# catniplab/vjf

Measured on AMD Instinct MI355X. Metric: trial-timesteps/sec, higher is better.
Workload: dtype f32

## Files before the change

include/vjf_hip.h:

```cpp
#ifndef VJF_HIP_H
#define VJF_HIP_H

#include <stdint.h>

#ifdef __cplusplus
extern "C" {
#endif

#define VJF_ABI_VERSION 1
#define VJF_MAX_HIDDEN 8

#define VJF_LIK_GAUSSIAN 0
#define VJF_LIK_POISSON 1

#define VJF_FLAG_SGD 1u
#define VJF_FLAG_UPDATE 2u
#define VJF_FLAG_WARM_UP 4u
#define VJF_FLAG_EXACT_NONFINITE 8u

#define VJF_STATUS_NONFINITE_RECON 1u
#define VJF_STATUS_NONFINITE_DYN 2u
#define VJF_STATUS_NONFINITE_ENT 4u
#define VJF_STATUS_RLS_FAILED 8u
#define VJF_STATUS_WAIT_RESIDENT 0x100u
// ... 137 lines not shown
int vjf_smooth_sample(const float* mu, const float* logvar, const float* u, const float* centroid, const float* logwidth,
                      const float* w_mean, const float* noise, const float* after, float* x,
                      int32_t T, int32_t S, int32_t B, int32_t n, int32_t d, int32_t dout, float state_var, void* stream);
int vjf_kstep_score_scratch_size(int32_t T, int32_t B, int32_t K, int32_t dout, int32_t dy, int64_t* bytes);
int vjf_kstep_score_plan(int32_t T, int32_t B, int32_t K, int32_t n, int32_t d, int32_t dout, int32_t dy, int64_t* lds_bytes,
                         int64_t* tiles, int64_t* tiles_per_chunk, int32_t* forms);
int vjf_kstep_score(const float* mu, const float* y, const float* u, const float* centroid, const float* logwidth,
                    const float* w_mean, const float* dec_W, const float* dec_b, double* sse_x, double* base_x, double* sse_y,
                    double* base_y, float* pred, void* scratch, int32_t T, int32_t B, int32_t K, int32_t n, int32_t d, int32_t dout,
                    int32_t dy, int32_t poisson, void* stream);
int vjf_ekf_plan(int32_t n, int32_t d, int32_t dout, int32_t dy, int64_t* lds_bytes);
int vjf_ekf(const float* y, const float* u, const uint8_t* observed, const float* centroid, const float* logwidth,
            const float* w_mean, const float* dec_W, const float* dec_b, const float* prior_mean, const float* prior_logvar,
            const float* prior_cov, float* mean, float* var, float* cov, float* loglik, float* cov_last, int32_t T, int32_t B,
            int32_t n, int32_t d, int32_t dout, int32_t dy, float state_var, float obs_var, void* stream);
int vjf_rls_scratch_size(int32_t B, int32_t n, int32_t dout, int64_t* bytes);
int vjf_blr_rls(const float* x, const float* target, const float* v, float shrink, const float* centroid,
                const float* logwidth, float* w_mean, float* w_chol, float* w_precision, float* w_pchol,
                void* scratch, uint32_t* status, int32_t B, int32_t n, int32_t d, int32_t dout, void* stream);

int vjf_kalman_scratch_size(int32_t B, int32_t n, int32_t dout, int64_t* bytes);
int vjf_blr_kalman(const float* x, const float* target, const float* v, float diffusion, const float* centroid,
                   const float* logwidth, float* w_mean, float* w_chol, void* scratch, uint32_t* status, int32_t B,
                   int32_t n, int32_t d, int32_t dout, void* stream);
int vjf_recognition_forward(const float* y, const float* u, const float* mu_s, const float* lv_s,
                            const float* const* rec_W, const float* const* rec_b, const float* mean_W,
                            const float* lv_W, const float* lv_b, float* mu_t, float* lv_t, int32_t B,
                            int32_t ydim, int32_t udim, int32_t xdim, int32_t n_hidden,
                            const int32_t* hidden, void* stream);
int vjf_recognition_forward_act(const float* y, const float* u, const float* mu_s, const float* lv_s,
// ... 16 lines not shown
```

vjf_amd/_native.py:

```python
import ctypes as C
import os

HERE = os.path.dirname(os.path.abspath(__file__))
_variant = os.environ.get("VJF_LIB", "")
LIB_PATH = os.path.join(HERE, f"libvjf_hip_{_variant}.so" if _variant.isalnum() else "libvjf_hip.so")

ABI_VERSION = 1
MAX_HIDDEN = 8
LIK_GAUSSIAN, LIK_POISSON = 0, 1
FLAG_SGD, FLAG_UPDATE, FLAG_WARM_UP, FLAG_EXACT_NONFINITE = 1, 2, 4, 8
STATUS_NONFINITE_RECON, STATUS_NONFINITE_DYN, STATUS_NONFINITE_ENT, STATUS_RLS_FAILED = 1, 2, 4, 8
STATUS_NOT_RESIDENT, STATUS_WAIT_MASK = 0x20000, 0x3ff00

SLOT_PRIOR_MEAN, SLOT_PRIOR_LOGVAR, SLOT_LIK_LOGVAR, SLOT_TR_LOGVAR, SLOT_CENTROID, SLOT_LOGWIDTH = range(6)
SLOT_REC_W0, SLOT_REC_B0 = 6, 7
SLOT_MEAN_W, SLOT_LV_W, SLOT_LV_B, SLOT_DEC_W, SLOT_DEC_B = 22, 23, 24, 25, 26
SLOT_W_MEAN, SLOT_W_CHOL, SLOT_W_PREC, SLOT_W_PCHOL, SLOT_SCALARS = 27, 28, 29, 30, 31
N_SLOTS = 32
SC_N_LIK, SC_N_TR, SC_LR_LIK, SC_LR_DEC, SC_LR_TR, SC_LR_REC, SC_FREEZE_DEC, SC_STATUS, SC_TRI_CLEAN, SC_SHRINK = range(10)
N_SCALARS = 16


ACT_TANH, ACT_RELU, ACT_LEAKY_RELU, ACT_ELU, ACT_SOFTPLUS, ACT_SIGMOID, ACT_HARDTANH = range(7)

# ... 48 lines not shown
    "vjf_forecast_ens_chunks": [_I, _I, _I, _I, _I, C.POINTER(_I), C.POINTER(_I)],
    "vjf_forecast_ens": [_P, C.c_int64] + [_P] * 16 + [_I] * 7 + [_P],
    "vjf_tangent_plan": [_I, _I, _I, _I, C.POINTER(_I), C.POINTER(C.c_int64)],
    "vjf_tangent_rollout": [_P] * 10 + [_I] * 8 + [_P],
    "vjf_fixed_points_plan": [_I, _I, _I, C.POINTER(C.c_int64)],
    "vjf_fixed_points": [_P] * 10 + [_I] * 5 + [_F, _F, _P],
    "vjf_smooth_plan": [_I, _I, _I, C.POINTER(C.c_int64)],
    "vjf_smooth": [_P] * 12 + [_I] * 5 + [_F, _P],
    "vjf_smooth_sample_plan": [_I, _I, _I, _I, C.POINTER(_I), C.POINTER(C.c_int64)],
    "vjf_smooth_sample": [_P] * 9 + [_I] * 6 + [_F, _P],
    "vjf_kstep_score_scratch_size": [_I, _I, _I, _I, _I, C.POINTER(C.c_int64)],
    "vjf_kstep_score_plan": [_I] * 7 + [C.POINTER(C.c_int64)] * 3 + [C.POINTER(_I)],
    "vjf_kstep_score": [_P] * 14 + [_I] * 8 + [_P],
    "vjf_ekf_plan": [_I, _I, _I, _I, C.POINTER(C.c_int64)],
    "vjf_ekf": [_P] * 16 + [_I] * 6 + [_F, _F, _P],
    "vjf_rls_scratch_size": [_I, _I, _I, C.POINTER(C.c_int64)],
    "vjf_blr_rls": [_P, _P, _P, _F, _P, _P, _P, _P, _P, _P, _P, _P, _I, _I, _I, _I, _P],
    "vjf_kalman_scratch_size": [_I, _I, _I, C.POINTER(C.c_int64)],
    "vjf_blr_kalman": [_P, _P, _P, _F, _P, _P, _P, _P, _P, _P, _I, _I, _I, _I, _P],
    "vjf_recognition_forward": [_P, _P, _P, _P, C.POINTER(_P), C.POINTER(_P), _P, _P, _P, _P, _P, _I, _I, _I, _I, _I,
                                C.POINTER(_I), _P],
    "vjf_recognition_forward_act": [_P, _P, _P, _P, C.POINTER(_P), C.POINTER(_P), _P, _P, _P, _P, _P, _I, _I, _I, _I, _I,
                                    C.POINTER(_I), C.POINTER(VjfActivation), _P],
    "vjf_gaussian_loss": [_P, _P, _P, _P, _P, _P, _I, _I, _P],
    "vjf_gaussian_entropy": [_P, _P, _I, _I, _P],
    "vjf_poisson_loss": [_P, _P, _P, _I, _I, _P],
    "vjf_linear_forward": [_P, _P, _P, _P, _I, _I, _I, _P],
}

_lib = None
# ... 64 lines not shown
```

vjf_amd/csrc/vjf_abi.hip:

```cpp
#include <hip/hip_runtime.h>
#include <hip/hip_ext.h>

#include <dlfcn.h>

#include <cstdarg>
#include <cstdio>
#include <cstdlib>
#include <cstring>
#include <ctime>
#include <atomic>
#include <mutex>
#include <new>
#include <string>
#include <type_traits>
#include <vector>

#include "../../include/vjf_hip.h"
#include "vjf_chol_blocks.h"
#include "vjf_chol_kernel.h"
#include "vjf_gram_kernel.h"
#include "vjf_handoff.h"
#include "vjf_mega_kernel.h"
#include "vjf_ops_kernels.h"
#include "vjf_plan.h"
// ... 634 lines not shown
        return fail(-20, "vjf_ekf: bad shape (T=%d B=%d n=%d d=%d dout=%d dy=%d state_var=%g obs_var=%g%s)", T, B, n, d, dout, dy,
                    (double)state_var, (double)obs_var, !prior_logvar == !prior_cov ? ", exactly one of prior_logvar / prior_cov is needed" : "");
    if (d > dout && !u) return fail(-21, "vjf_ekf: u is required when d > dout");
    const EkfPlan p = ekf_plan(n, d, dout, dy, fc_env_on("VJF_FC_CENTROID_LDS"), fc_env_on("VJF_EKF_DECODER_LDS"));
    if (!p.fits)
        return fail(-11, "vjf_ekf: n=%d, d=%d, dout=%d beyond %s", n, d, dout,
                    dout > VJF_EKF_MAXDOUT ? "dout <= 32 (VJF_EKF_MAXDOUT)" : "one workgroup's LDS");
    VjfEkfArgs a{};
    a.y = y; a.u = d > dout ? u : nullptr; a.obs = observed; a.c = centroid; a.logw = logwidth; a.w = w_mean; a.dec_W = dec_W;
    a.dec_b = dec_b; a.prior_mean = prior_mean; a.prior_lv = prior_logvar; a.prior_cov = prior_cov; a.mean = mean; a.var = var;
    a.cov = cov; a.ll = loglik; a.cov_last = cov_last; a.T = T; a.B = B; a.n = n; a.d = d; a.dout = dout; a.dy = dy; a.q = state_var;
    a.r = obs_var;
    return ekf_run(a, p, (hipStream_t)stream);
}

int vjf_rls_scratch_size(int32_t B, int32_t n, int32_t dout, int64_t* bytes) {
    if (!bytes || B < 1 || n < 1 || dout < 1) return fail(-20, "vjf_rls_scratch_size: bad argument");
    *bytes = (int64_t)rls_carve(B, n, dout, nullptr).total;
    return 0;
}

int vjf_blr_rls(const float* x, const float* target, const float* v, float shrink, const float* centroid, const float* logwidth,
                float* w_mean, float* w_chol, float* w_precision, float* w_pchol, void* scratch, uint32_t* status, int32_t B,
                int32_t n, int32_t d, int32_t dout, void* stream) {
    if (!x || !target || !v || !centroid || !logwidth || !w_mean || !w_chol || !w_precision || !w_pchol || !scratch)
        return fail(-1, "vjf_blr_rls: null tensor");
    if (B < 1 || n < 1 || d < 1 || dout < 1) return fail(-20, "vjf_blr_rls: bad shape");
    return rls_update("vjf_blr_rls", "RLS kernel", vjf_rls_kernel, scratch, x, target, centroid, logwidth, B, n, d, dout, stream, [&](VjfRlsArgs& a, const RlsStats& st) {
        a.Pm = w_precision; a.Wm = w_mean; a.Wc = w_chol; a.Lm = w_pchol;
        a.G = st.red + st.P.red_G; a.FDX = st.red + st.P.red_FDX; a.v = v; a.work = (float*)(st.ws + st.c.work); a.status = status;
// ... 74 lines not shown
```

vjf_amd/csrc/vjf_mega_trial.h:

```cpp
#pragma once
#include "vjf_mega_common.h"

template <bool RLS, bool ACT = false>
__device__ __forceinline__ void vjf_mega_trial(const VjfPlan& P, const VjfMegaArgs& A, float* smem, const int wg, const VjfAct act = VjfAct{}) {
    constexpr int LD = VJF_MG_LD, NW = VJF_MG_WAVES, NT = VJF_MG_THREADS, TR = VJF_MG_TR;
    constexpr bool VSPLIT = RLS && !ACT;
    const int tid0 = threadIdx.x;
    const int dz = P.dz, dy = P.dy, du = P.du, n = P.n, din = P.din, dxu = P.dxu;
    const float* S = A.state;
    float* SCW = A.state + P.off[VJF_SLOT_SCALARS];
    const bool do_sgd = RLS || (A.flags & VJF_FLAG_SGD) != 0u, do_upd = RLS || (A.flags & VJF_FLAG_UPDATE) != 0u;
    const bool warm = !RLS && (A.flags & VJF_FLAG_WARM_UP) != 0u;
    constexpr bool mode_rls = RLS;
    const bool gated = RLS || do_sgd || do_upd;
    const bool want_resid = !RLS && do_upd && warm;
    const bool use_mom = !RLS && A.n_mom > 0;
    const unsigned m_dy = mg_magic(dy), m_dz = mg_magic(dz), m_du = mg_magic(du > 0 ? du : 1);
    const VjfMegaTrialLds Lo = vjf_mega_trial_lds<false>(P, A.lds_floats);
    const bool tl = Lo.theta != 0;
    float* s_cen = smem + Lo.cen; float* s_iw = smem + Lo.iw;
    float* s_in = smem + Lo.in; float* s_xu = smem + Lo.xu; float* s_phi = smem + Lo.phi; float* s_act = smem + Lo.act;
    float* s_dd = smem + Lo.dd;
    float* s_mu = smem + Lo.mu; float* s_lv = smem + Lo.lv; float* s_xt = smem + Lo.xt; float* s_e2 = smem + Lo.e2; float* s_pm = smem + Lo.pm;
    float* s_dmu = smem + Lo.dmu; float* s_dlv = smem + Lo.dlv; float* s_dx = smem + Lo.dx;
// ... 457 lines not shown
                else if (tid < ly + le) tp = en + min((tid - ly) * 32, nbn * dz - 1);
                else if (tid < ly + 2 * le) tp = en + sz + min((tid - ly - le) * 32, nbn * dz - 1);
                if (tp) touch = *tp;
            }
            if (tid == 0 && !replay && mode_rls) {
                float v = 0.f;
                for (int bb = 0; bb < TR; ++bb) v += s_sc[bb * RS_N + RS_SDX2];
                s_wg[RS_SDX2] += v;
                if (last) vjf_st_wt(early + (size_t)16 * ldn + RS_SDX2, s_wg[RS_SDX2]);
            }
            if (first) VJF_MG_STAMP(26);
            const bool fuse_fwd = first && last && !replay && !rls_in && s_wg[15] != 0.f;
            if (last && !replay && !fuse_fwd && mode_rls) vjf_wg_signal_wt(cnt + MG_C_FWD, tid);
            if (first) VJF_MG_STAMP(4);
            if (last) { VJF_MG_STAMPX(28, -1); VJF_MG_STAMPW(1); }
            float4 wv_late[2];
            bool warm_late = false;
            if (first && !rls_in) {
                if (!vjf_wg_wait_sc1<RLS ? VJF_POLL_SLEEP : VJF_POLL_SLEEP_LITE>(cnt + MG_C_PDONE, (unsigned)t * npost, tid, SCW + VJF_SC_STATUS, (A.flags & VJF_FLAG_HANDOFF_ACQUIRE) != 0u))
                    vjf_status_or(SCW + VJF_SC_STATUS, VJF_STATUS_RLS_FAILED | VJF_STATUS_WAIT_K1);
                if (vjf_abort_wg()) return;
                sig = vjf_ld_sc1(S + P.off[VJF_SLOT_TR_LOGVAR]);
                tri = vjf_ld_sc1(SCW + VJF_SC_TRI_CLEAN) != 0.f;
                if (fuse_fwd) {
                    vjf_chaos(tid, cnt + MG_C_FWD, 2);
                    asm volatile("s_waitcnt vmcnt(0)" ::: "memory");
                    __syncthreads();
                    if (tid == 0) __hip_atomic_fetch_add(cnt + MG_C_FWD, 1u, __ATOMIC_RELAXED, __HIP_MEMORY_SCOPE_AGENT);
                }
                mg_warm_issue(A.xt, P.n * P.n, wg, tid, wv_late);
// ... 20 lines not shown
            if (last && tid == 0 && !replay && mode_rls) __hip_atomic_fetch_add(cnt + MG_C_K1, 1u, __ATOMIC_RELAXED, __HIP_MEMORY_SCOPE_AGENT);
            if (RLS) moments_b();
            if (do_sgd)
            for (int e = tid; e < TR * (dz + 1); e += NT) {
                const int j = e >> 5, b = e & 31;
                if (b < nb) {
                    float* sv = A.pmsave + (size_t)(b0 + b) * (dz + 1) + j;
                    if (!replay) *sv = j < dz ? s_pm[j * LD + b] : s_plv[b];
                    else if (j < dz) s_pm[j * LD + b] = *sv;
                    else s_plv[b] = *sv;
                }
            }
            if (replay) { __syncthreads(); MG_PHASE(); }
            if (first) VJF_MG_STAMP(10);
            if (first) { VJF_MG_STAMP(6); VJF_MG_STAMPW(3); }
            {
                constexpr int LPT = NT / TR;
                const int b = tid / LPT, s = tid % LPT;
                const bool ok = b < nb;
                float lrec = 0.f, ssey = 0.f;
                if (P.lik == VJF_LIK_GAUSSIAN) {
                    const float p = expf(-0.5f * rho), e = expf(-rho);
                    for (int i = s; i < dy; i += LPT) {
                        const float seed = vjf_gauss_recon(s_in[i * LD + b], s_py[i * LD + b], rho, p, e, lrec, ssey);
                        s_dpy[i * LD + b] = (ok && m_r) ? seed : 0.f;
                    }
                } else {
                    for (int i = s; i < dy; i += LPT) {
                        const float seed = vjf_poisson_recon(s_in[i * LD + b], s_py[i * LD + b], lrec, ssey);
                        s_dpy[i * LD + b] = (ok && m_r) ? seed : 0.f;
                    }
                }
                lrec = group_sum<LPT>(lrec);
                ssey = group_sum<LPT>(ssey);
                float ldyn = 0.f, ent = 0.f, rsd = 0.f;
                {
                    const float p = expf(-0.5f * sig), e = expf(-sig), plv = s_plv[b];
                    for (int j = s; j < dz; j += LPT) {
                        if (want_resid) { const float r = s_dx[j * LD + b] - s_dmu[j * LD + b]; rsd = fmaf(r, r, rsd); }
                        const VjfDynSeed sd = vjf_dyn_term(s_pm[j * LD + b], s_mu[j * LD + b], s_lv[j * LD + b], plv, sig, p, e, !warm && m_d, m_h, ldyn, ent);
                        s_dmu[j * LD + b] = ok ? sd.dmu : 0.f;
                        s_dlv[j * LD + b] = ok ? sd.dlv : 0.f;
                    }
                }
                ldyn = group_sum<LPT>(ldyn);
                ent = group_sum<LPT>(ent);
                if (want_resid) rsd = group_sum<LPT>(rsd);
                if (s == 0) {
                    s_sc[b * RS_N + RS_RESID] = ok ? rsd : 0.f;
                    s_sc[b * RS_N + RS_LRECON] = ok ? lrec : 0.f;
                    s_sc[b * RS_N + RS_LDYN] = ok ? ldyn : 0.f;
                    s_sc[b * RS_N + RS_ENT] = ok ? ent : 0.f;
                    s_sc[b * RS_N + RS_SSEY] = ok ? ssey : 0.f;
                }
            }
            __syncthreads(); MG_PHASE();
            if (first) VJF_MG_STAMP(31);
#ifdef VJF_EXPERIMENT_SLOW_TRIAL
            { const unsigned long long t0_ = wall_clock64(); while (wall_clock64() - t0_ < VJF_EXPERIMENT_SLOW_TRIAL) __builtin_amdgcn_s_sleep(1); }
#endif
            if ((tid < RS_SDX2 || (tid == RS_RESID && want_resid)) && !replay) {
                float v = 0.f;
                for (int bb = 0; bb < TR; ++bb) v += s_sc[bb * RS_N + tid];
                s_wg[tid] += v;
            }
            if (do_sgd) {
            int gbase = 0;
            auto grad_tensor = [&](const float* D, int M, const float* Bact, int Kin, int blkid) {
                int b_off, b_ldm, b_rows;
                mg_slab_block(P, blkid, b_off, b_ldm, b_rows);
                const int ntm = (M + 15) >> 4, ntj = (Kin + 1 + 15) >> 4;
                const unsigned mj = mg_magic(ntj);
                for (int q = (wave - gbase) & (NW - 1); q < ntm * ntj; q += NW) {
                    const int tm = mg_div(q, mj), tj = q - tm * ntj;
                    mg_grad_tile(D, M, tm * 16, Bact, Kin, tj * 16, s_one, s_zero, late + b_off, b_ldm, b_rows, first, lane);
                }
                gbase += ntm * ntj;
            };
            {
                const float* C = S + P.off[VJF_SLOT_DEC_W];
                const int mt = (dz + 15) >> 4;
                float* s_kp = compact ? s_py : s_dd;
                const int rows_av = compact ? dy : Lo.nd * P.hmax;
                const int nslb = min(NW / mt, rows_av / (16 * mt));
                if (nslb >= 2) {
                    if (wave < mt * nslb) {
                        const int tt = wave / nslb, sl = wave - tt * nslb;
                        const int per = (((dy + 3) >> 2) + nslb - 1) / nslb * 4;
                        vjf_f32x4 acc0 = {0.f, 0.f, 0.f, 0.f}, acc1 = {0.f, 0.f, 0.f, 0.f};
                        if (tl) mg_mma2_lds<true>(acc0, acc1, smem + Lo.th_dec, Lo.th_ldd, dz, tt * 16, s_dpy, sl * per, min(dy, (sl + 1) * per), lane);
                        else mg_mma2(acc0, acc1, C, dz, dz, tt * 16, s_dpy, sl * per, min(dy, (sl + 1) * per), lane);
                        float* pr = s_kp + (size_t)((sl * mt + tt) * 16 + 4 * (lane >> 4)) * LD + (lane & 15);
#pragma unroll
                        for (int r = 0; r < 4; ++r) { pr[r * LD] = acc0[r]; pr[r * LD + 16] = acc1[r]; }
                    }
                    __syncthreads(); MG_PHASE();
                    for (int e = tid; e < TR * dz; e += NT) {
                        const int j = e >> 5, b = e & 31;
                        float a = 0.f;
                        for (int sl = 0; sl < nslb; ++sl) a += s_kp[(size_t)((sl * mt + (j >> 4)) * 16 + (j & 15)) * LD + b];
                        s_dmu[j * LD + b] += a;
                        s_dlv[j * LD + b] = fmaf(a * s_e2[j * LD + b], 0.5f * expf(0.5f * s_lv[j * LD + b]), s_dlv[j * LD + b]);
                    }
                } else
                for (int tt = wave; tt < mt; tt += NW) {
                    vjf_f32x4 acc0 = {0.f, 0.f, 0.f, 0.f}, acc1 = {0.f, 0.f, 0.f, 0.f};
                    if (tl) mg_mma2_lds<true>(acc0, acc1, smem + Lo.th_dec, Lo.th_ldd, dz, tt * 16, s_dpy, 0, dy, lane);
                    else mg_mma2(acc0, acc1, C, dz, dz, tt * 16, s_dpy, 0, dy, lane);
#pragma unroll
                    for (int r = 0; r < 4; ++r) {
                        const int j = tt * 16 + 4 * (lane >> 4) + r;
                        if (j < dz) {
#pragma unroll
                            for (int g = 0; g < 2; ++g) {
                                const int b = 16 * g + (lane & 15);
// ... 125 lines not shown
```

vjf_amd/csrc/vjf_post_kernel.h:

```cpp
#pragma once
#include <hip/hip_runtime.h>
#include "vjf_handoff.h"
#include "vjf_plan.h"
#include "vjf_chol_kernel.h"
#include "vjf_trial_mfma_kernel.h"

#define VJF_POST_THREADS 512
#define VJF_POST_KPAR 4
#define VJF_POST_LDB 33
#define VJF_POST_LDX 17
#define VJF_RESID_BLOCKS 64

struct VjfPostArgs {
    float* state;
    const float* dinv;
    const float* lscr;
    const float* gbuf;
    const unsigned* flags;
    unsigned epoch;
    float* status;
    const unsigned* k1_done;
    unsigned k1_target;
    unsigned* started;
    unsigned* done;
// ... 15 lines not shown
#define VJF_POST_STAMP(i)                                                                   \
    do {                                                                                    \
        if (A.stamps && solve && tid == 0) {                                                \
            unsigned long long t_;                                                          \
            asm volatile("s_memrealtime %0\n\ts_waitcnt lgkmcnt(0)" : "=s"(t_)::"memory");      \
            A.stamps[((it_epoch & 7u) << 5) * (A.nsteps > 0 ? 1 : 0) + (i)] = t_;              \
        }                                                                                   \
    } while (0)

static inline size_t vjf_post_inv_lds_bytes(const VjfPlan& P) {
    const int nbl = (P.n + 31) / 32;
    return ((size_t)nbl * 32 * VJF_POST_LDB + (size_t)nbl * 32 * VJF_POST_LDX + 32 * VJF_POST_LDX + 64 + 16 + 16) * 4;
}
static inline size_t vjf_post_lds_bytes(const VjfPlan& P) {
    const int nbl = (P.n + 31) / 32;
    return ((size_t)(nbl * (nbl - 1) / 2 + nbl) * 32 * VJF_POST_LDB + (size_t)nbl * 32 * VJF_POST_LDX + 32 * VJF_POST_LDX + 64 + 16 + 16) * 4;
}

template <class FA>
__device__ __forceinline__ void post_mma32(vjf_f32x4& acc, const float* Bs, int lane, FA fa) {
    const int i = lane & 15, kk = lane >> 4;
    float a[8], b[8];
#pragma unroll
    for (int s = 0; s < 8; ++s) { a[s] = fa(i, 4 * s + kk); b[s] = Bs[(4 * s + kk) * VJF_POST_LDX + i]; }
    __builtin_amdgcn_sched_barrier(0);
    vjf_f32x4 acc1 = {0.f, 0.f, 0.f, 0.f};
#pragma unroll
    for (int s = 0; s < 8; s += 2) {
        acc = __builtin_amdgcn_mfma_f32_16x16x4f32(a[s], b[s], acc, 0, 0, 0);
        acc1 = __builtin_amdgcn_mfma_f32_16x16x4f32(a[s + 1], b[s + 1], acc1, 0, 0, 0);
    }
// ... 41 lines not shown

__device__ __forceinline__ void vjf_rls_post_body(const VjfPlan& P, const VjfPostArgs& A, float* lds, int* s_dead, const unsigned it_epoch,
                                                  const float* it_red, const unsigned it_k1_target, const unsigned it_prep_target,
                                                  const bool it_first, const int role, const int bix) {
    int tid = threadIdx.x;
    asm volatile("" : "+v"(tid));
    const int lane = tid & 63, wave = tid >> 6;
    const int n = P.n, dz = P.dz, nbl = (n + 31) / 32, ntri = nbl * (nbl + 1) / 2, nlow = ntri - nbl;
    const bool solve = role == 2 || bix == 2 * nbl;
    const bool col_only = role == 1;
    constexpr int LB = VJF_POST_LDB, LX = VJF_POST_LDX;
    float* s_L = lds;
    float* s_D = s_L + (size_t)(col_only ? nbl - 1 : nlow) * 32 * LB;
    float* s_x = s_D + (size_t)(col_only ? 1 : nbl) * 32 * LB;
    float* s_y = s_x + (size_t)nbl * 32 * LX;
    int* s_tab = reinterpret_cast<int*>(s_y + 32 * LX);
    int* s_ctl = s_tab + 64;
    auto leave = [&]() {
        vjf_chaos(tid, A.done, 2);
        asm volatile("s_waitcnt vmcnt(0)" ::: "memory");
        __syncthreads();
        if (A.stamps && !solve && tid == 0) {
            unsigned long long t_;
            asm volatile("s_memrealtime %0\n\ts_waitcnt lgkmcnt(0)" : "=s"(t_)::"memory");
            atomicMax(A.stamps + ((it_epoch & 7u) << 5) * (A.nsteps > 0 ? 1 : 0) + 22, t_);
        }
        if (tid == 0 && A.done) __hip_atomic_fetch_add(A.done, 1u, __ATOMIC_RELAXED, __HIP_MEMORY_SCOPE_AGENT);
    };
    const float* S = A.state;
    const __amdgpu_buffer_rsrc_t r_L = vjf_rsrc(A.lscr, (size_t)n * n), r_dinv = vjf_rsrc(A.dinv, (size_t)nbl * 1024);
    const int j0 = solve ? 0 : bix >> 1;
    const int c0 = solve ? 0 : 16 * (bix & 1);
    auto tri = [](int bi, int bj) { return bi * (bi - 1) / 2 + bj; };
    auto lblk = [&](int bi, int bj) { return s_L + (size_t)(col_only ? bi - bj - 1 : tri(bi, bj)) * 32 * LB; };
    auto dblk = [&](int k) { return s_D + (size_t)(col_only ? 0 : k) * 32 * LB; };

    if (tid == 0 && A.started && it_first) __hip_atomic_fetch_add(A.started, 1u, __ATOMIC_RELAXED, __HIP_MEMORY_SCOPE_AGENT);
    float pre_sdx2 = 0.f, pre_old = 0.f, pre_tot = 1.f;
    double pre_scale = 0.0;
    VJF_POST_STAMP(16);
    if (tid < ntri) {
        int bi = 0;
        while ((bi + 1) * (bi + 2) / 2 <= tid) ++bi;
        s_tab[32 + tid] = (bi << 8) | (tid - bi * (bi + 1) / 2);
    }
    if (!solve)
        for (int e = tid; e < nbl * 32 * 16; e += VJF_POST_THREADS) {
            const int r = e >> 4, c = e & 15;
            s_x[r * LX + c] = (r == j0 * 32 + c0 + c) ? 1.f : 0.f;
        }
    __syncthreads();

    float gpre[4][16], fpre[8];
    unsigned wbits[4];
    {
        const int c = lane & 31, h = lane >> 5;
#pragma unroll
        for (int q = 0; q < 4; ++q) {
            const int t = wave + 8 * q;
            unsigned wq = 0u;
            if (solve && t < ntri) {
                const int code = s_tab[32 + t], bi = code >> 8, bj = code & 255;
#pragma unroll
                for (int r = 0; r < 16; ++r) {
                    const int gi = bi * 32 + (r & 3) + 8 * (r >> 2) + 4 * h, gj = bj * 32 + c;
                    wq |= ((gi >= n || gj > gi) ? 0u : (gj == gi ? 1u : 2u)) << (2 * r);
                }
            }
            wbits[q] = wq;
        }
    }
    auto prefetch_G = [&]() {
        const float* G = it_red + P.red_G;
        const int c = lane & 31, h = lane >> 5;
#pragma unroll
        for (int q = 0; q < 4; ++q) {
            const int code = s_tab[32 + min(wave + 8 * q, ntri - 1)];
            const int bi = code >> 8, bj = code & 255;
#pragma unroll
            for (int r = 0; r < 16; ++r) {
                const int gi = min(bi * 32 + (r & 3) + 8 * (r >> 2) + 4 * h, n - 1), gj = min(bj * 32 + c, n - 1);
                gpre[q][r] = vjf_ld_sc1(G + (size_t)gi * n + gj);
            }
        }
    };
    auto prefetch_rest = [&]() {
        pre_sdx2 = vjf_ld_sc1(it_red + P.red_SC + RS_SDX2);
        const float sig = vjf_ld_sc1(S + P.off[VJF_SLOT_TR_LOGVAR]);
        const float Bf = (float)A.B_total;
        pre_old = vjf_running_old_share(sig, vjf_ld_sc1(S + P.off[VJF_SLOT_SCALARS] + VJF_SC_N_TR), VJF_TR_VAR_CAP, Bf, pre_tot);
        pre_scale = 1.0 / ((double)Bf * (double)P.dz);
        const float* FDX = it_red + P.red_FDX;
#pragma unroll
        for (int q = 0; q < 8; ++q) {
            const int e = tid + q * VJF_POST_THREADS, r = min(e >> 4, n - 1), cc = min(e & 15, dz - 1);
            fpre[q] = vjf_ld_sc1(FDX + r * dz + cc);
        }
    };
    auto prefetch_tail = [&]() { prefetch_G(); prefetch_rest(); };

    const int tile = wave & 1, grp = wave >> 1;
    const int xr = 4 * (lane >> 4), xc = lane & 15;
    int bad = 0;
    bool g_there = A.prep_count == nullptr;
    auto wait_g = [&]() {
        if (g_there) return;
        g_there = true;
        if (!vjf_wg_wait(A.prep_count, it_prep_target, tid, A.status)) { vjf_status_or(A.status, VJF_STATUS_RLS_FAILED | VJF_STATUS_WAIT_G); *s_dead = 1; }
    };
    auto stage_column = [&](int k) {
        const int nb = nbl - k;
        float4 v[4];
        const int r = (tid >> 3) & 31, c4 = (tid & 7) * 4, bh = tid >> 8;
#pragma unroll
// ... 126 lines not shown
                }
            }
            if (A.xt) {
                const int gc0 = j0 * 32 + c0;
                for (int e = tid; e < (n - first) * 4; e += VJF_POST_THREADS) {
                    const int i = first + (e >> 2), q = (e & 3) * 4;
                    if (gc0 + q < n) {
                        vjf_f32x4 o = {s_x[i * LX + q], s_x[i * LX + q + 1], s_x[i * LX + q + 2], s_x[i * LX + q + 3]};
                        vjf_st4_wt(A.xt + (size_t)i * n + gc0 + q, o);
                    }
                }
            }
            leave();
            return;
        }
        for (int k = nbl - 1; k >= 0; --k) {
            vjf_f32x4 w = {0.f, 0.f, 0.f, 0.f};
            if (wave < 2) {
                const float* Db = s_D + (size_t)k * 32 * LB;
                post_mma32(w, s_x + (size_t)k * 32 * LX, lane, [&](int i, int m) { return Db[m * LB + 16 * wave + i]; });
#pragma unroll
                for (int r = 0; r < 4; ++r) s_y[(16 * wave + xr + r) * LX + xc] = w[r];
            }
            __syncthreads();
            if (wave < 2) {
#pragma unroll
                for (int r = 0; r < 4; ++r) s_x[(k * 32 + 16 * wave + xr + r) * LX + xc] = w[r];
            }
            for (int i = k - 1 - grp; i >= 0; i -= VJF_POST_THREADS / 128) {
                const float* Lb = s_L + (size_t)tri(k, i) * 32 * LB;
                float* xt = s_x + ((size_t)i * 32 + 16 * tile + xr) * LX + xc;
                vjf_f32x4 acc;
#pragma unroll
                for (int r = 0; r < 4; ++r) acc[r] = xt[r * LX];
                post_mma32(acc, s_y, lane, [&](int ii, int m) { return -Lb[m * LB + 16 * tile + ii]; });
#pragma unroll
                for (int r = 0; r < 4; ++r) xt[r * LX] = acc[r];
            }
            __syncthreads();
        }
        VJF_POST_STAMP(19);
    }
    auto store_W = [&]() {
        float* Wm = A.state + P.off[VJF_SLOT_W_MEAN];
        for (int e = tid; e < n * 16; e += VJF_POST_THREADS) {
            const int r = e >> 4, c = e & 15;
            if (c < dz) __hip_atomic_store(Wm + r * dz + c, s_x[r * LX + c], __ATOMIC_RELAXED, __HIP_MEMORY_SCOPE_AGENT);
        }
    };
    if (!failed && !k1_late) store_W();
    if (!A.fold_sigma) { leave(); return; }
    {
// ... 3 lines not shown
            if (tid == 0) { __builtin_amdgcn_fence(__ATOMIC_ACQUIRE, "agent"); asm volatile("s_waitcnt vmcnt(0)" ::: "memory"); }
            __syncthreads();
            const float* Wold = A.state + P.off[VJF_SLOT_W_MEAN];
            for (int e = tid; e < nbl * 32 * 16; e += VJF_POST_THREADS) {
                const int r = e >> 4, c = e & 15;
                s_x[r * LX + c] = (r < n && c < dz) ? Wold[(size_t)r * dz + c] : 0.f;
            }
            prefetch_tail();
            if (A.undo_P) {
                float* Pm = A.state + P.off[VJF_SLOT_W_PREC];
                const float* G = it_red + P.red_G;
                const float inv_v = expf(-S[P.off[VJF_SLOT_TR_LOGVAR]]);
                const float lam = vjf_shrink_of(S[P.off[VJF_SLOT_SCALARS] + VJF_SC_SHRINK]);
                for (int e = tid; e < n * n; e += VJF_POST_THREADS) vjf_st_wt(Pm + e, __fdiv_rn(fmaf(-G[e], inv_v, Pm[e]), lam));
            }
        }
        __syncthreads();
        VJF_POST_STAMP(20);
#ifdef VJF_EXPERIMENT_SLOW_RLS
        { const unsigned long long t0_ = wall_clock64(); while (wall_clock64() - t0_ < VJF_EXPERIMENT_SLOW_RLS) __builtin_amdgcn_s_sleep(1); }
#endif
        double part = 0.0;
        const int c = lane & 31, h = lane >> 5;
#pragma unroll
        for (int q = 0; q < 4; ++q) {
            const int t = wave + 8 * q;
            if (t < ntri) {
                const int code = s_tab[32 + t], bi = code >> 8, bj = code & 255;
                vjf_f32x16 acc;
#pragma unroll
                for (int r = 0; r < 16; ++r) acc[r] = 0.f;
                float wa[8], wb[8];
#pragma unroll
                for (int k = 0; k < 8; ++k) {
                    wa[k] = s_x[(bi * 32 + c) * LX + 2 * k + h];
                    wb[k] = s_x[(bj * 32 + c) * LX + 2 * k + h];
                }
#pragma unroll
                for (int k = 0; k < 8; ++k)
                    if (2 * k < dz) acc = __builtin_amdgcn_mfma_f32_32x32x2f32(wa[k], wb[k], acc, 0, 0, 0);
                double tp = 0.0;
#pragma unroll
                for (int r = 0; r < 16; ++r) {
                    const float wgt = (float)((wbits[q] >> (2 * r)) & 3u);
                    tp += (double)((wgt * gpre[q][r]) * acc[r]);
                }
                part += tp;
            }
        }
#pragma unroll
        for (int q = 0; q < 8; ++q) {
            const int e = tid + q * VJF_POST_THREADS, r = e >> 4, cc = e & 15;
            if (r < n && cc < dz) part -= 2.0 * (double)s_x[r * LX + cc] * (double)fpre[q];
        }

#pragma unroll
        for (int o = 32; o > 0; o >>= 1) part += __shfl_xor(part, o, 64);
        if (lane == 0) s_p[wave] = part;
        __syncthreads();
        if (tid == 0) {
            double t = 0.0;
            for (int w = 0; w < VJF_POST_THREADS / 64; ++w) t += s_p[w];
            t += (double)pre_sdx2;
// ... 197 lines not shown
```

Baseline: 83.07 million.

## Overlap back-substitution with W·Wᵀ trace tiles and hoist recon seeding

Restructures the post kernel's block back-substitution. Two waves now run the critical diagonal chain: they compute the next y block early into a double buffer, and the other six waves perform the off-diagonal updates in parallel. The sigma-fold W·Wᵀ trace tiles are dealt statically to waves and computed as soon as their column block is final, with per-tile partials kept in LDS, instead of as a separate pass afterward. In the mega-trial kernel, recon seed computation and decoder-gradient partials are moved earlier so they run before the warm/rls section. The cost is extra LDS, more complex scheduling, and a new tile-deal ABI helper.

```diff
diff --git a/include/vjf_hip.h b/include/vjf_hip.h
--- a/include/vjf_hip.h
+++ b/include/vjf_hip.h
@@ -175,6 +175,7 @@
             const float* w_mean, const float* dec_W, const float* dec_b, const float* prior_mean, const float* prior_logvar,
             const float* prior_cov, float* mean, float* var, float* cov, float* loglik, float* cov_last, int32_t T, int32_t B,
             int32_t n, int32_t d, int32_t dout, int32_t dy, float state_var, float obs_var, void* stream);
+int vjf_post_tile_deal(int32_t nbl, int32_t* owner, int32_t* step, int32_t* slots);
 int vjf_rls_scratch_size(int32_t B, int32_t n, int32_t dout, int64_t* bytes);
 int vjf_blr_rls(const float* x, const float* target, const float* v, float shrink, const float* centroid,
                 const float* logwidth, float* w_mean, float* w_chol, float* w_precision, float* w_pchol,
diff --git a/vjf_amd/_native.py b/vjf_amd/_native.py
--- a/vjf_amd/_native.py
+++ b/vjf_amd/_native.py
@@ -86,6 +86,7 @@
     "vjf_kstep_score": [_P] * 14 + [_I] * 8 + [_P],
     "vjf_ekf_plan": [_I, _I, _I, _I, C.POINTER(C.c_int64)],
     "vjf_ekf": [_P] * 16 + [_I] * 6 + [_F, _F, _P],
+    "vjf_post_tile_deal": [_I, C.POINTER(_I), C.POINTER(_I), C.POINTER(_I)],
     "vjf_rls_scratch_size": [_I, _I, _I, C.POINTER(C.c_int64)],
     "vjf_blr_rls": [_P, _P, _P, _F, _P, _P, _P, _P, _P, _P, _P, _P, _I, _I, _I, _I, _P],
     "vjf_kalman_scratch_size": [_I, _I, _I, C.POINTER(C.c_int64)],
diff --git a/vjf_amd/csrc/vjf_abi.hip b/vjf_amd/csrc/vjf_abi.hip
--- a/vjf_amd/csrc/vjf_abi.hip
+++ b/vjf_amd/csrc/vjf_abi.hip
@@ -672,6 +672,22 @@
     return ekf_run(a, p, (hipStream_t)stream);
 }
 
+int vjf_post_tile_deal(int32_t nbl, int32_t* owner, int32_t* step, int32_t* slots) {
+    if (!owner || !step || !slots || nbl < 1 || nbl > VJF_POST_MAXBLK) return fail(-20, "vjf_post_tile_deal: bad argument");
+    for (int bi = 0; bi < nbl; ++bi)
+        for (int bj = 0; bj <= bi; ++bj) {
+            owner[bi * (bi + 1) / 2 + bj] = vjf_post_deal_owner(nbl, bi, bj);
+            step[bi * (bi + 1) / 2 + bj] = bj;
+        }
+    for (int w = 0; w < VJF_POST_WAVES; ++w) {
+        int code[VJF_POST_SLOTS];
+        const int cnt = vjf_post_deal_slots(nbl, w, code);
+        if (cnt > VJF_POST_SLOTS) return fail(-11, "vjf_post_tile_deal: wavefront %d has %d tiles at nbl=%d", w, cnt, nbl);
+        for (int q = 0; q < VJF_POST_SLOTS; ++q) slots[w * VJF_POST_SLOTS + q] = code[q];
+    }
+    return 0;
+}
+
 int vjf_rls_scratch_size(int32_t B, int32_t n, int32_t dout, int64_t* bytes) {
     if (!bytes || B < 1 || n < 1 || dout < 1) return fail(-20, "vjf_rls_scratch_size: bad argument");
     *bytes = (int64_t)rls_carve(B, n, dout, nullptr).total;
diff --git a/vjf_amd/csrc/vjf_mega_trial.h b/vjf_amd/csrc/vjf_mega_trial.h
--- a/vjf_amd/csrc/vjf_mega_trial.h
+++ b/vjf_amd/csrc/vjf_mega_trial.h
@@ -5,6 +5,7 @@
 __device__ __forceinline__ void vjf_mega_trial(const VjfPlan& P, const VjfMegaArgs& A, float* smem, const int wg, const VjfAct act = VjfAct{}) {
     constexpr int LD = VJF_MG_LD, NW = VJF_MG_WAVES, NT = VJF_MG_THREADS, TR = VJF_MG_TR;
     constexpr bool VSPLIT = RLS && !ACT;
+    constexpr bool PRE = RLS && !ACT;
     const int tid0 = threadIdx.x;
     const int dz = P.dz, dy = P.dy, du = P.du, n = P.n, din = P.din, dxu = P.dxu;
     const float* S = A.state;
@@ -495,6 +496,66 @@
             if (last && !replay && !fuse_fwd && mode_rls) vjf_wg_signal_wt(cnt + MG_C_FWD, tid);
             if (first) VJF_MG_STAMP(4);
             if (last) { VJF_MG_STAMPX(28, -1); VJF_MG_STAMPW(1); }
+            auto recon_seeds = [&]() {
+                constexpr int LPT = NT / TR;
+                const int b = tid / LPT, s = tid % LPT;
+                const bool ok = b < nb;
+                float lrec = 0.f, ssey = 0.f;
+                if (P.lik == VJF_LIK_GAUSSIAN) {
+                    const float p = expf(-0.5f * rho), e = expf(-rho);
+                    for (int i = s; i < dy; i += LPT) {
+                        const float seed = vjf_gauss_recon(s_in[i * LD + b], s_py[i * LD + b], rho, p, e, lrec, ssey);
+                        s_dpy[i * LD + b] = (ok && m_r) ? seed : 0.f;
+                    }
+                } else {
+                    for (int i = s; i < dy; i += LPT) {
+                        const float seed = vjf_poisson_recon(s_in[i * LD + b], s_py[i * LD + b], lrec, ssey);
+                        s_dpy[i * LD + b] = (ok && m_r) ? seed : 0.f;
+                    }
+                }
+                lrec = group_sum<LPT>(lrec);
+                ssey = group_sum<LPT>(ssey);
+                if (s == 0) {
+                    s_sc[b * RS_N + RS_LRECON] = ok ? lrec : 0.f;
+                    s_sc[b * RS_N + RS_SSEY] = ok ? ssey : 0.f;
+                }
+            };
+            const int kp_mt = (dz + 15) >> 4;
+            float* s_kp = compact ? s_py : s_dd;
+            const int nslb = min(NW / kp_mt, (compact ? dy : Lo.nd * P.hmax) / (16 * kp_mt));
+            auto dpyc_partials = [&]() {
+                if (wave < kp_mt * nslb) {
+                    const float* C = S + P.off[VJF_SLOT_DEC_W];
+                    const int tt = wave / nslb, sl = wave - tt * nslb;
+                    const int per = (((dy + 3) >> 2) + nslb - 1) / nslb * 4;
+                    vjf_f32x4 acc0 = {0.f, 0.f, 0.f, 0.f}, acc1 = {0.f, 0.f, 0.f, 0.f};
+                    if (tl) mg_mma2_lds<true>(acc0, acc1, smem + Lo.th_dec, Lo.th_ldd, dz, tt * 16, s_dpy, sl * per, min(dy, (sl + 1) * per), lane);
+                    else mg_mma2(acc0, acc1, C, dz, dz, tt * 16, s_dpy, sl * per, min(dy, (sl + 1) * per), lane);
+                    float* pr = s_kp + (size_t)((sl * kp_mt + tt) * 16 + 4 * (lane >> 4)) * LD + (lane & 15);
+#pragma unroll
+                    for (int r = 0; r < 4; ++r) { pr[r * LD] = acc0[r]; pr[r * LD + 16] = acc1[r]; }
+                }
+            };
+            auto dpyc_sum = [&](int j, int b) {
+                float a = 0.f;
+                for (int sl = 0; sl < nslb; ++sl) a += s_kp[(size_t)((sl * kp_mt + (j >> 4)) * 16 + (j & 15)) * LD + b];
+                return a;
+            };
+            const bool pre = PRE && tl && Lo.part != Lo.dpy;
+            const bool pre_kp = pre && do_sgd && nslb >= 2;
+            if (pre) {
+                recon_seeds();
+                if (pre_kp) {
+                    __syncthreads(); MG_PHASE();
+                    dpyc_partials();
+                    __syncthreads(); MG_PHASE();
+                    for (int e = tid; e < TR * dz; e += NT) {
+                        const int j = e >> 5, b = e & 31;
+                        s_dx[j * LD + b] = dpyc_sum(j, b);
+                    }
+                    if (s_kp == s_part && !(first && !rls_in)) { __syncthreads(); MG_PHASE(); }
+                }
+            }
             float4 wv_late[2];
             bool warm_late = false;
             if (first && !rls_in) {
@@ -545,25 +606,11 @@
             if (replay) { __syncthreads(); MG_PHASE(); }
             if (first) VJF_MG_STAMP(10);
             if (first) { VJF_MG_STAMP(6); VJF_MG_STAMPW(3); }
+            if (!pre) recon_seeds();
             {
                 constexpr int LPT = NT / TR;
                 const int b = tid / LPT, s = tid % LPT;
                 const bool ok = b < nb;
-                float lrec = 0.f, ssey = 0.f;
-                if (P.lik == VJF_LIK_GAUSSIAN) {
-                    const float p = expf(-0.5f * rho), e = expf(-rho);
-                    for (int i = s; i < dy; i += LPT) {
-                        const float seed = vjf_gauss_recon(s_in[i * LD + b], s_py[i * LD + b], rho, p, e, lrec, ssey);
-                        s_dpy[i * LD + b] = (ok && m_r) ? seed : 0.f;
-                    }
-                } else {
-                    for (int i = s; i < dy; i += LPT) {
-                        const float seed = vjf_poisson_recon(s_in[i * LD + b], s_py[i * LD + b], lrec, ssey);
-                        s_dpy[i * LD + b] = (ok && m_r) ? seed : 0.f;
-                    }
-                }
-                lrec = group_sum<LPT>(lrec);
-                ssey = group_sum<LPT>(ssey);
                 float ldyn = 0.f, ent = 0.f, rsd = 0.f;
                 {
                     const float p = expf(-0.5f * sig), e = expf(-sig), plv = s_plv[b];
@@ -579,10 +626,8 @@
                 if (want_resid) rsd = group_sum<LPT>(rsd);
                 if (s == 0) {
                     s_sc[b * RS_N + RS_RESID] = ok ? rsd : 0.f;
-                    s_sc[b * RS_N + RS_LRECON] = ok ? lrec : 0.f;
                     s_sc[b * RS_N + RS_LDYN] = ok ? ldyn : 0.f;
                     s_sc[b * RS_N + RS_ENT] = ok ? ent : 0.f;
-                    s_sc[b * RS_N + RS_SSEY] = ok ? ssey : 0.f;
                 }
             }
             __syncthreads(); MG_PHASE();
@@ -610,26 +655,12 @@
             };
             {
                 const float* C = S + P.off[VJF_SLOT_DEC_W];
-                const int mt = (dz + 15) >> 4;
-                float* s_kp = compact ? s_py : s_dd;
-                const int rows_av = compact ? dy : Lo.nd * P.hmax;
-                const int nslb = min(NW / mt, rows_av / (16 * mt));
+                const int mt = kp_mt;
                 if (nslb >= 2) {
-                    if (wave < mt * nslb) {
-                        const int tt = wave / nslb, sl = wave - tt * nslb;
-                        const int per = (((dy + 3) >> 2) + nslb - 1) / nslb * 4;
-                        vjf_f32x4 acc0 = {0.f, 0.f, 0.f, 0.f}, acc1 = {0.f, 0.f, 0.f, 0.f};
-                        if (tl) mg_mma2_lds<true>(acc0, acc1, smem + Lo.th_dec, Lo.th_ldd, dz, tt * 16, s_dpy, sl * per, min(dy, (sl + 1) * per), lane);
-                        else mg_mma2(acc0, acc1, C, dz, dz, tt * 16, s_dpy, sl * per, min(dy, (sl + 1) * per), lane);
-                        float* pr = s_kp + (size_t)((sl * mt + tt) * 16 + 4 * (lane >> 4)) * LD + (lane & 15);
-#pragma unroll
-                        for (int r = 0; r < 4; ++r) { pr[r * LD] = acc0[r]; pr[r * LD + 16] = acc1[r]; }
-                    }
-                    __syncthreads(); MG_PHASE();
+                    if (!pre_kp) { dpyc_partials(); __syncthreads(); MG_PHASE(); }
                     for (int e = tid; e < TR * dz; e += NT) {
                         const int j = e >> 5, b = e & 31;
-                        float a = 0.f;
-                        for (int sl = 0; sl < nslb; ++sl) a += s_kp[(size_t)((sl * mt + (j >> 4)) * 16 + (j & 15)) * LD + b];
+                        const float a = pre_kp ? s_dx[j * LD + b] : dpyc_sum(j, b);
                         s_dmu[j * LD + b] += a;
                         s_dlv[j * LD + b] = fmaf(a * s_e2[j * LD + b], 0.5f * expf(0.5f * s_lv[j * LD + b]), s_dlv[j * LD + b]);
                     }
diff --git a/vjf_amd/csrc/vjf_post_deal.h b/vjf_amd/csrc/vjf_post_deal.h
--- /dev/null
+++ b/vjf_amd/csrc/vjf_post_deal.h
@@ -0,0 +1,28 @@
+#pragma once
+
+#define VJF_POST_WAVES 8
+#define VJF_POST_SLOTS 5
+#define VJF_POST_MAXBLK 7
+
+__host__ __device__ inline int vjf_post_deal_updates(int k) { return k >= 1 ? 2 * (k - 1) : 0; }
+
+__host__ __device__ inline int vjf_post_deal_owner(int nbl, int bi, int bj) {
+    (void)nbl;
+    if (bj == 0) return bi;
+    return 2 + (vjf_post_deal_updates(bj) + (bi - bj)) % (VJF_POST_WAVES - 2);
+}
+
+__host__ __device__ inline int vjf_post_deal_slots(int nbl, int wave, int code[VJF_POST_SLOTS]) {
+    int cnt = 0;
+#pragma unroll
+    for (int q = 0; q < VJF_POST_SLOTS; ++q) code[q] = -1;
+    for (int bj = nbl - 1; bj >= 0; --bj)
+        for (int bi = bj; bi < nbl; ++bi)
+            if (vjf_post_deal_owner(nbl, bi, bj) == wave) {
+#pragma unroll
+                for (int q = 0; q < VJF_POST_SLOTS; ++q)
+                    if (q == cnt) code[q] = (bi << 8) | bj;
+                ++cnt;
+            }
+    return cnt;
+}
diff --git a/vjf_amd/csrc/vjf_post_kernel.h b/vjf_amd/csrc/vjf_post_kernel.h
--- a/vjf_amd/csrc/vjf_post_kernel.h
+++ b/vjf_amd/csrc/vjf_post_kernel.h
@@ -2,6 +2,7 @@
 #include <hip/hip_runtime.h>
 #include "vjf_handoff.h"
 #include "vjf_plan.h"
+#include "vjf_post_deal.h"
 #include "vjf_chol_kernel.h"
 #include "vjf_trial_mfma_kernel.h"
 
@@ -53,7 +54,8 @@
 }
 static inline size_t vjf_post_lds_bytes(const VjfPlan& P) {
     const int nbl = (P.n + 31) / 32;
-    return ((size_t)(nbl * (nbl - 1) / 2 + nbl) * 32 * VJF_POST_LDB + (size_t)nbl * 32 * VJF_POST_LDX + 32 * VJF_POST_LDX + 64 + 16 + 16) * 4;
+    return ((size_t)(nbl * (nbl - 1) / 2 + nbl) * 32 * VJF_POST_LDB + (size_t)nbl * 32 * VJF_POST_LDX + 32 * VJF_POST_LDX + 64 + 16 + 16) * 4
+           + (size_t)3 * 32 * VJF_POST_LDX * 4 + (size_t)(nbl * (nbl + 1) / 2) * 64 * 8;
 }
 
 template <class FA>
@@ -125,8 +127,10 @@
     float* s_D = s_L + (size_t)(col_only ? nbl - 1 : nlow) * 32 * LB;
     float* s_x = s_D + (size_t)(col_only ? 1 : nbl) * 32 * LB;
     float* s_y = s_x + (size_t)nbl * 32 * LX;
-    int* s_tab = reinterpret_cast<int*>(s_y + 32 * LX);
-    int* s_ctl = s_tab + 64;
+    int* s_ctl = reinterpret_cast<int*>(s_y + 32 * LX) + 64;
+    float* s_y1 = reinterpret_cast<float*>(s_ctl + 32);
+    float* s_rp = s_y1 + 32 * LX;
+    double* s_tp = reinterpret_cast<double*>(s_rp + 2 * 32 * LX);
     auto leave = [&]() {
         vjf_chaos(tid, A.done, 2);
         asm volatile("s_waitcnt vmcnt(0)" ::: "memory");
@@ -150,11 +154,6 @@
     float pre_sdx2 = 0.f, pre_old = 0.f, pre_tot = 1.f;
     double pre_scale = 0.0;
     VJF_POST_STAMP(16);
-    if (tid < ntri) {
-        int bi = 0;
-        while ((bi + 1) * (bi + 2) / 2 <= tid) ++bi;
-        s_tab[32 + tid] = (bi << 8) | (tid - bi * (bi + 1) / 2);
-    }
     if (!solve)
         for (int e = tid; e < nbl * 32 * 16; e += VJF_POST_THREADS) {
             const int r = e >> 4, c = e & 15;
@@ -162,16 +161,19 @@
         }
     __syncthreads();
 
-    float gpre[4][16], fpre[8];
-    unsigned wbits[4];
+    float gpre[VJF_POST_SLOTS][16], fpre[8];
+    int tcode[VJF_POST_SLOTS];
+#pragma unroll
+    for (int q = 0; q < VJF_POST_SLOTS; ++q) tcode[q] = -1;
+    if (solve) vjf_post_deal_slots(nbl, __builtin_amdgcn_readfirstlane(wave), tcode);
+    unsigned wbits[VJF_POST_SLOTS];
     {
         const int c = lane & 31, h = lane >> 5;
 #pragma unroll
-        for (int q = 0; q < 4; ++q) {
-            const int t = wave + 8 * q;
+        for (int q = 0; q < VJF_POST_SLOTS; ++q) {
             unsigned wq = 0u;
-            if (solve && t < ntri) {
-                const int code = s_tab[32 + t], bi = code >> 8, bj = code & 255;
+            if (tcode[q] >= 0) {
+                const int code = tcode[q], bi = code >> 8, bj = code & 255;
 #pragma unroll
                 for (int r = 0; r < 16; ++r) {
                     const int gi = bi * 32 + (r & 3) + 8 * (r >> 2) + 4 * h, gj = bj * 32 + c;
@@ -183,10 +185,12 @@
     }
     auto prefetch_G = [&]() {
         const float* G = it_red + P.red_G;
-        const int c = lane & 31, h = lane >> 5;
-#pragma unroll
-        for (int q = 0; q < 4; ++q) {
-            const int code = s_tab[32 + min(wave + 8 * q, ntri - 1)];
+        int ln = lane;
+        asm volatile("" : "+v"(ln));
+        const int c = ln & 31, h = ln >> 5;
+#pragma unroll
+        for (int q = 0; q < VJF_POST_SLOTS; ++q) {
+            const int code = max(tcode[q], 0);
             const int bi = code >> 8, bj = code & 255;
 #pragma unroll
             for (int r = 0; r < 16; ++r) {
@@ -209,6 +213,30 @@
         }
     };
     auto prefetch_tail = [&]() { prefetch_G(); prefetch_rest(); };
+    auto wwt_tile = [&](const int q, const int kcur, const float* ycur) {
+        const int c = lane & 31, h = lane >> 5;
+        const int code = tcode[q], bi = code >> 8, bj = code & 255;
+        const float* Wa = (bi == kcur ? ycur : s_x + (size_t)bi * 32 * LX) + c * LX + h;
+        const float* Wb = (bj == kcur ? ycur : s_x + (size_t)bj * 32 * LX) + c * LX + h;
+        vjf_f32x16 acc;
+#pragma unroll
+        for (int r = 0; r < 16; ++r) acc[r] = 0.f;
+        float wa[8], wb[8];
+#pragma unroll
+        for (int k = 0; k < 8; ++k) { wa[k] = Wa[2 * k]; wb[k] = Wb[2 * k]; }
+#pragma unroll
+        for (int k = 0; k < 8; ++k)
+            if (2 * k < dz) acc = __builtin_amdgcn_mfma_f32_32x32x2f32(wa[k], wb[k], acc, 0, 0, 0);
+        unsigned wq = wbits[q];
+        asm volatile("" : "+v"(wq));
+        double tp = 0.0;
+#pragma unroll
+        for (int r = 0; r < 16; ++r) {
+            const float wgt = (float)((wq >> (2 * r)) & 3u);
+            tp += (double)((wgt * gpre[q][r]) * acc[r]);
+        }
+        s_tp[(size_t)(bi * (bi + 1) / 2 + bj) * 64 + lane] = tp;
+    };
 
     const int tile = wave & 1, grp = wave >> 1;
     const int xr = 4 * (lane >> 4), xc = lane & 15;
@@ -365,28 +393,61 @@
             leave();
             return;
         }
+        const bool fold = A.fold_sigma != 0;
+        vjf_f32x4 w = {0.f, 0.f, 0.f, 0.f};
+        if (wave < 2) {
+            const int k = nbl - 1;
+            const float* Db = s_D + (size_t)k * 32 * LB;
+            post_mma32(w, s_x + (size_t)k * 32 * LX, lane, [&](int i, int m) { return Db[m * LB + 16 * wave + i]; });
+            float* yk = (k & 1) ? s_y1 : s_y;
+#pragma unroll
+            for (int r = 0; r < 4; ++r) yk[(16 * wave + xr + r) * LX + xc] = w[r];
+        }
+        __syncthreads();
         for (int k = nbl - 1; k >= 0; --k) {
-            vjf_f32x4 w = {0.f, 0.f, 0.f, 0.f};
+            const float* yk = (k & 1) ? s_y1 : s_y;
             if (wave < 2) {
-                const float* Db = s_D + (size_t)k * 32 * LB;
-                post_mma32(w, s_x + (size_t)k * 32 * LX, lane, [&](int i, int m) { return Db[m * LB + 16 * wave + i]; });
-#pragma unroll
-                for (int r = 0; r < 4; ++r) s_y[(16 * wave + xr + r) * LX + xc] = w[r];
-            }
-            __syncthreads();
-            if (wave < 2) {
 #pragma unroll
                 for (int r = 0; r < 4; ++r) s_x[(k * 32 + 16 * wave + xr + r) * LX + xc] = w[r];
-            }
-            for (int i = k - 1 - grp; i >= 0; i -= VJF_POST_THREADS / 128) {
-                const float* Lb = s_L + (size_t)tri(k, i) * 32 * LB;
-                float* xt = s_x + ((size_t)i * 32 + 16 * tile + xr) * LX + xc;
-                vjf_f32x4 acc;
-#pragma unroll
-                for (int r = 0; r < 4; ++r) acc[r] = xt[r * LX];
-                post_mma32(acc, s_y, lane, [&](int ii, int m) { return -Lb[m * LB + 16 * tile + ii]; });
-#pragma unroll
-                for (int r = 0; r < 4; ++r) xt[r * LX] = acc[r];
+                if (k > 0) {
+                    const float* Lb = s_L + (size_t)tri(k, k - 1) * 32 * LB;
+                    float* rp = s_rp + (size_t)wave * 32 * LX;
+#pragma unroll
+                    for (int t2 = 0; t2 < 2; ++t2) {
+                        const float* xt = s_x + ((size_t)(k - 1) * 32 + 16 * t2 + xr) * LX + xc;
+                        vjf_f32x4 acc;
+#pragma unroll
+                        for (int r = 0; r < 4; ++r) acc[r] = xt[r * LX];
+                        post_mma32(acc, yk, lane, [&](int ii, int m) { return -Lb[m * LB + 16 * t2 + ii]; });
+#pragma unroll
+                        for (int r = 0; r < 4; ++r) rp[(16 * t2 + xr + r) * LX + xc] = acc[r];
+                    }
+                    __builtin_amdgcn_wave_barrier();
+                    const float* Db = s_D + (size_t)(k - 1) * 32 * LB;
+                    w = vjf_f32x4{0.f, 0.f, 0.f, 0.f};
+                    post_mma32(w, rp, lane, [&](int i, int m) { return Db[m * LB + 16 * wave + i]; });
+                    float* yn = (k & 1) ? s_y : s_y1;
+#pragma unroll
+                    for (int r = 0; r < 4; ++r) yn[(16 * wave + xr + r) * LX + xc] = w[r];
+                }
+            } else {
+                const int nupd = vjf_post_deal_updates(k);
+                for (int u = wave - 2; u < nupd; u += VJF_POST_WAVES - 2) {
+                    const int i = k - 2 - (u >> 1), t2 = u & 1;
+                    const float* Lb = s_L + (size_t)tri(k, i) * 32 * LB;
+                    float* xt = s_x + ((size_t)i * 32 + 16 * t2 + xr) * LX + xc;
+                    vjf_f32x4 acc;
+#pragma unroll
+                    for (int r = 0; r < 4; ++r) acc[r] = xt[r * LX];
+                    post_mma32(acc, yk, lane, [&](int ii, int m) { return -Lb[m * LB + 16 * t2 + ii]; });
+#pragma unroll
+                    for (int r = 0; r < 4; ++r) xt[r * LX] = acc[r];
+                }
+            }
+            if (fold) {
+#pragma unroll
+                for (int q = 0; q < VJF_POST_SLOTS; ++q)
+                    if (tcode[q] >= 0 && (tcode[q] & 255) == k) wwt_tile(q, k, yk);
             }
             __syncthreads();
         }
@@ -420,39 +481,23 @@
                 const float lam = vjf_shrink_of(S[P.off[VJF_SLOT_SCALARS] + VJF_SC_SHRINK]);
                 for (int e = tid; e < n * n; e += VJF_POST_THREADS) vjf_st_wt(Pm + e, __fdiv_rn(fmaf(-G[e], inv_v, Pm[e]), lam));
             }
-        }
-        __syncthreads();
+            __syncthreads();
+        }
         VJF_POST_STAMP(20);
 #ifdef VJF_EXPERIMENT_SLOW_RLS
         { const unsigned long long t0_ = wall_clock64(); while (wall_clock64() - t0_ < VJF_EXPERIMENT_SLOW_RLS) __builtin_amdgcn_s_sleep(1); }
 #endif
+        if (failed) {
+#pragma unroll
+            for (int q = 0; q < VJF_POST_SLOTS; ++q)
+                if (tcode[q] >= 0) wwt_tile(q, -1, s_x);
+            __syncthreads();
+        }
         double part = 0.0;
-        const int c = lane & 31, h = lane >> 5;
 #pragma unroll
         for (int q = 0; q < 4; ++q) {
             const int t = wave + 8 * q;
-            if (t < ntri) {
-                const int code = s_tab[32 + t], bi = code >> 8, bj = code & 255;
-                vjf_f32x16 acc;
-#pragma unroll
-                for (int r = 0; r < 16; ++r) acc[r] = 0.f;
-                float wa[8], wb[8];
-#pragma unroll
-                for (int k = 0; k < 8; ++k) {
-                    wa[k] = s_x[(bi * 32 + c) * LX + 2 * k + h];
-                    wb[k] = s_x[(bj * 32 + c) * LX + 2 * k + h];
-                }
-#pragma unroll
-                for (int k = 0; k < 8; ++k)
-                    if (2 * k < dz) acc = __builtin_amdgcn_mfma_f32_32x32x2f32(wa[k], wb[k], acc, 0, 0, 0);
-                double tp = 0.0;
-#pragma unroll
-                for (int r = 0; r < 16; ++r) {
-                    const float wgt = (float)((wbits[q] >> (2 * r)) & 3u);
-                    tp += (double)((wgt * gpre[q][r]) * acc[r]);
-                }
-                part += tp;
-            }
+            if (t < ntri) part += s_tp[(size_t)t * 64 + lane];
         }
 #pragma unroll
         for (int q = 0; q < 8; ++q) {
```

After: 81.28 million. 2.2% lower.
